# mct10/Speech-Vecalign

Measured on AMD Instinct MI355X. Metric: aligned doc-pairs/sec, higher is better.
Workload: dtype bf16; 1 GPU; synthetic 4096x4096 d=1024 bf16 embeddings, 4 overlap layers/side, 10 alignment types, band 14, coarse-to-fine (max_size_full_dp=300), 1024 doc-pairs per GPU per step; pipeline=1, N=4096, M=4096, d=1024, overlaps=4, parallelism=dp1 (pairs sharded, no collective)

## Files before the change

### include/svx.h

```cpp
#ifndef SVX_H
#define SVX_H

#include <stdint.h>

#ifdef __cplusplus
extern "C" {
#endif

typedef struct svx_ctx svx_ctx;

enum svx_dtype { SVX_F32 = 0, SVX_F16 = 1, SVX_BF16 = 2 };

enum svx_status {
    SVX_OK = 0,
    SVX_ERR_ARG = 1,
    SVX_ERR_OVERLAPS = 2,
    SVX_ERR_HIP = 3,
    SVX_ERR_TRACEBACK = 4,
    SVX_ERR_NOMEM = 5,
    SVX_ERR_EXTEND = 6,
    SVX_ERR_PATH = 7,
    SVX_ERR_BP = 8
};

#define SVX_MAX_LEVELS 16
#define SVX_MAX_TYPES 128
#define SVX_MAX_DIM 2048

int svx_create(int device_id, svx_ctx **out);
int svx_destroy(svx_ctx *ctx);
int svx_set_stream(svx_ctx *ctx, void *hip_stream);
int svx_synchronize(svx_ctx *ctx);
const char *svx_last_error(const svx_ctx *ctx);
const char *svx_version(void);
int64_t svx_scratch_bytes(const svx_ctx *ctx);


int svx_dense_costs(svx_ctx *ctx, const float *vecs0, int k0, int s0, const float *vecs1, int k1, int s1, int d,
                    const float *norm0, const float *norm1, int offset0, int offset1, float *costs);

int svx_dense_dp(svx_ctx *ctx, const float *cost, int s0, int s1, float pen, double *csum, int32_t *bp);

int svx_score_path(svx_ctx *ctx, const int32_t *xx, const int32_t *yy, int64_t n, const float *norm1,
                   const float *norm2, const float *vecs1, int rows1, const float *vecs2, int rows2, int d, float *out);

int svx_sparse_costs(svx_ctx *ctx, const float *vecs0, int k0, int xsize, const float *vecs1, int k1, int ysize,
                     int d, const float *norms0, const float *norms1, const int32_t *path, int A,
                     const int32_t *types_host, int T, int width_over2, float *costs, int32_t *b_offset);

int svx_sparse_dp(svx_ctx *ctx, const float *costs, const int32_t *b_offset_in, int A, int B,
                  const int32_t *types_host, int T, double del_penalty, int x_in_size, int y_in_size,
                  double *csum, int32_t *xp, int32_t *yp, int32_t *b_offset_out);


int svx_make_norm1(svx_ctx *ctx, float *vecs, int64_t rows, int d);

int svx_downsample(svx_ctx *ctx, const float *vecs, int k, int n, int d, float *half);

int svx_compute_norms(svx_ctx *ctx, const float *vecs0, int k0, int n0, const float *vecs1, int k1, int n1, int d,
                      const int32_t *idx, int samples_per_overlap, float *norms0);

int svx_del_penalty(svx_ctx *ctx, const float *scores, int64_t n, double frac, double *del_penalty);

int svx_dense_traceback(svx_ctx *ctx, const int32_t *bp, int s0, int s1, int32_t *align, int32_t *count);

int svx_sparse_traceback(svx_ctx *ctx, const double *csum, const int32_t *xp, const int32_t *yp,
                         const int32_t *b_offset_out, int a_out, int B, int xsize, int ysize, int32_t *align,
                         double *scores, int32_t *count);

int svx_search_path(svx_ctx *ctx, const int32_t *align, const int32_t *n_align, int upsample, int size0,
                    int size1, int32_t *path, int32_t *path_len);

int svx_gather_rows(svx_ctx *ctx, const void *table, int64_t n_rows, int d, int dtype, const int32_t *idx, int64_t n_out,
                    void *out);


int svx_mt19937_choice(uint32_t *key, int32_t *pos, int64_t n, int64_t size, int32_t *out);

int64_t svx_norm_index_count(int n, int m, int k0, int k1, int max_size_full_dp, int num_samps_for_norm, int have_norms0,
                             int have_norms1);
int64_t svx_knob_index_count(int n, int m, int max_size_full_dp, int costs_sample_size);

int svx_draw_indices(uint32_t *key, int32_t *pos, int n, int m, int k0, int k1, int max_size_full_dp, int costs_sample_size,
                     int num_samps_for_norm, int have_norms0, int have_norms1, int32_t *norm_idx, int32_t *knob_idx);

int svx_candidate_table(const char *seg_path, const char *cat_path, const char *ignore_path, int max_overlaps, int32_t *table,
                        int cap_lines, int32_t *n_lines, int64_t *n_candidates, char *err, int err_cap);

int64_t svx_format_alignments(const int32_t *rows, const double *scores, int64_t n, char *out, int64_t cap);


#define SVX_MARGIN_RATIO 0
#define SVX_MARGIN_DISTANCE 1
#define SVX_MARGIN_ABSOLUTE 2

int svx_unit_rows(svx_ctx *ctx, const void *rows, int dtype, int64_t n, int d, void *out, int out_dtype);

int svx_knn_mean_sim(svx_ctx *ctx, const void *queries, int q_dtype, int64_t n, const void *db, int db_dtype,
                     int64_t n_db, int d, int k, float *mean_sim);

int svx_knn_topk_merge(svx_ctx *ctx, const void *queries, int q_dtype, int64_t n, const void *db, int db_dtype,
                       int64_t n_db, int d, int k, float *topk, int first, float *mean_sim);

int svx_knn_search(svx_ctx *ctx, const void *queries, int q_dtype, int64_t n, const void *db, int db_dtype,
                   int64_t n_db, int d, int k, int64_t id_base, float *sims, int64_t *ids, int first);

int svx_margin_scores(svx_ctx *ctx, const void *x, const void *y, int dtype, int64_t n, int d, const float *mean_xy,
                      const float *mean_yx, int margin, float *scores);


int svx_knn_list_means(svx_ctx *ctx, const float *sims, int64_t n, int k, float *mean);

int svx_margin_candidates(svx_ctx *ctx, const float *sims, const int64_t *ids, int64_t n, int k, const float *mean_q,
                          const float *mean_db, int64_t n_db, int64_t id_base, int margin, float *scores, int64_t *best_id,
                          float *best_score);

int64_t svx_mine_greedy(const int64_t *order, int64_t n_cand, const int64_t *src, const int64_t *tgt, int64_t n_src,
                        int64_t n_tgt, int64_t *out);


typedef struct svx_align_params {
    int32_t dtype;
    int32_t d;
    int32_t n_types;
    int32_t types[2 * SVX_MAX_TYPES];
    int32_t width_over2;
    int32_t max_size_full_dp;
    int32_t costs_sample_size;
    int32_t num_samps_for_norm;
    double del_percentile_frac;
    int32_t search_mode;
    int32_t reserved0;
} svx_align_params;

#define SVX_SEARCH_COARSE_TO_FINE 0
// ... 54 lines not shown
```

### speech-vecalign_amd/csrc/svx_api.hip

```cpp
#include <stdarg.h>
#include <stdio.h>
#include <stdlib.h>
#include <string.h>

#include <chrono>
#include <functional>
#include <memory>
#include <type_traits>
#include <vector>

#include "svx_common.h"

static char g_err[512] = "";

int svx_fail(svx_ctx* ctx, int code, const char* fmt, ...) {
    char* dst = ctx ? ctx->err : g_err;
    va_list ap;
    va_start(ap, fmt);
    vsnprintf(dst, 512, fmt, ap);
    va_end(ap);
    return code;
}

static const char* kStageNames[] = {"pyr0",       "pyrN",     "pyr_aux",      "knob_scoresN", "knob",      "dense_costs",
// ... 277 lines not shown
        if (x < 1 || y < 1 || x > 100 || y > 100) return svx_fail(ctx, SVX_ERR_ARG, "alignment type (%d,%d): sizes must be >= 1", x, y);
        out->x[t] = (int8_t)x;
        out->y[t] = (int8_t)y;
        if (x + y > out->maxstep) out->maxstep = x + y;
    }
    out->x[T] = 0; out->y[T] = 1;
    out->x[T + 1] = 1; out->y[T + 1] = 0;
    return SVX_OK;
}

static int check_dim(svx_ctx* ctx, int d) {
    if (d <= 0 || d % 8 != 0 || d > SVX_MAX_DIM)
        return svx_fail(ctx, SVX_ERR_ARG, "embedding dimension %d: must be a positive multiple of 8, at most %d", d, SVX_MAX_DIM);
    return SVX_OK;
}

#define NEED(ctx, cond, ...) \
    do { if (!(cond)) return svx_fail(ctx, SVX_ERR_ARG, __VA_ARGS__); } while (0)

extern "C" {

int svx_dense_costs(svx_ctx* ctx, const float* vecs0, int k0, int s0, const float* vecs1, int k1, int s1, int d,
                    const float* norm0, const float* norm1, int offset0, int offset1, float* costs) {
    NEED(ctx, ctx && vecs0 && vecs1 && norm0 && norm1 && costs, "svx_dense_costs: null argument");
    NEED(ctx, k0 > offset0 && k1 > offset1 && offset0 >= 0 && offset1 >= 0, "svx_dense_costs: offsets (%d,%d) outside %d/%d layers", offset0, offset1, k0, k1);
    int rc = check_dim(ctx, d);
    if (rc) return rc;
    return svxl_dense_costs(ctx, vecs0 + (size_t)offset0 * s0 * d, s0, vecs1 + (size_t)offset1 * s1 * d, s1, d,
                            norm0 + (size_t)offset0 * s0, norm1 + (size_t)offset1 * s1, offset0 + 1, offset1 + 1, costs);
}

int svx_dense_dp(svx_ctx* ctx, const float* cost, int s0, int s1, float pen, double* csum, int32_t* bp) {
    NEED(ctx, ctx && bp && (cost || s0 == 0 || s1 == 0), "svx_dense_dp: null argument");
    NEED(ctx, s0 >= 0 && s1 >= 0, "svx_dense_dp: negative size");
    return svxl_dense_dp(ctx, cost, s0, s1, pen, csum, bp);
}

int svx_score_path(svx_ctx* ctx, const int32_t* xx, const int32_t* yy, int64_t n, const float* norm1, const float* norm2,
                   const float* vecs1, int rows1, const float* vecs2, int rows2, int d, float* out) {
    NEED(ctx, ctx && xx && yy && norm1 && norm2 && vecs1 && vecs2 && out, "svx_score_path: null argument");
    NEED(ctx, rows1 > 0 && rows2 > 0, "svx_score_path: empty vecs");
    int rc = check_dim(ctx, d);
    if (rc) return rc;
    return svxl_score_path(ctx, xx, yy, n, norm1, norm2, vecs1, rows1, vecs2, rows2, d, out);
}

int svx_sparse_costs(svx_ctx* ctx, const float* vecs0, int k0, int xsize, const float* vecs1, int k1, int ysize, int d,
                     const float* norms0, const float* norms1, const int32_t* path, int A, const int32_t* types_host, int T,
                     int width_over2, float* costs, int32_t* b_offset) {
    NEED(ctx, ctx && vecs0 && vecs1 && norms0 && norms1 && path && b_offset && (costs || T == 0), "svx_sparse_costs: null argument");
    NEED(ctx, width_over2 >= 1 && A >= 0, "svx_sparse_costs: bad width/path length");
    int rc = check_dim(ctx, d);
    if (rc) return rc;
    SvxTypes ty;
    rc = make_types(ctx, types_host, T, &ty);
    if (rc) return rc;
    int mx = 0, my = 0;
    for (int t = 0; t < T; t++) { if (ty.x[t] > mx) mx = ty.x[t]; if (ty.y[t] > my) my = ty.y[t]; }
    if (mx > k0) return svx_fail(ctx, SVX_ERR_OVERLAPS, "%d x overlaps requrested (via alignment_types), but vecs0 only has %d", mx, k0);
    if (my > k1) return svx_fail(ctx, SVX_ERR_OVERLAPS, "%d y overlaps requrested (via alignment_types), but vecs1 only has %d", my, k1);
    rc = arena_reserve(ctx, 256);
    if (rc) return rc;
    int* status = reinterpret_cast<int*>(ctx->arena);
    SVX_HIP(ctx, hipMemsetAsync(status, 0, sizeof(int), ctx->stream));
    rc = svxl_band_costs(ctx, vecs0, k0, xsize, vecs1, k1, ysize, d, SVX_F32, nullptr, nullptr, norms0, norms1, path, A, ty,
                         width_over2, costs, b_offset, status);
    if (rc) return rc;
    int hs = 0;
    SVX_HIP(ctx, hipMemcpyAsync(&hs, status, sizeof(int), hipMemcpyDeviceToHost, ctx->stream));
    SVX_HIP(ctx, hipStreamSynchronize(ctx->stream));
    if (hs != 0) return svx_fail(ctx, hs, "search path is not a unit-step lattice path starting at (0,0)");
    return SVX_OK;
}

int svx_sparse_dp(svx_ctx* ctx, const float* costs, const int32_t* b_offset_in, int A, int B, const int32_t* types_host,
                  int T, double del_penalty, int x_in_size, int y_in_size, double* csum, int32_t* xp, int32_t* yp,
                  int32_t* b_offset_out) {
    NEED(ctx, ctx && b_offset_in && csum && xp && yp && b_offset_out && (costs || T == 0), "svx_sparse_dp: null argument");
    NEED(ctx, A >= 1 && B >= 1, "svx_sparse_dp: empty cost band");
    SvxTypes ty;
    int rc = make_types(ctx, types_host, T, &ty);
    if (rc) return rc;
    return svxl_sparse_dp(ctx, costs, b_offset_in, A, B, ty, del_penalty, x_in_size, y_in_size, csum, xp, yp, b_offset_out);
}

int svx_make_norm1(svx_ctx* ctx, float* vecs, int64_t rows, int d) {
    NEED(ctx, ctx && (vecs || rows == 0), "svx_make_norm1: null argument");
    int rc = check_dim(ctx, d);
    if (rc) return rc;
    return svxl_make_norm1(ctx, vecs, rows, d);
}

int svx_downsample(svx_ctx* ctx, const float* vecs, int k, int n, int d, float* half) {
    NEED(ctx, ctx && vecs && (half || n < 2), "svx_downsample: null argument");
    int rc = check_dim(ctx, d);
    if (rc) return rc;
    const int h = n / 2;
    if (h <= 0 || k <= 0) return SVX_OK;
    const int nblk = (h + SVX_PYR_SLOTS - 1) / SVX_PYR_SLOTS;
    Bump b;
    size_t o_part = b.take((size_t)k * nblk * d * sizeof(float));
    size_t o_mean = b.take((size_t)k * d * sizeof(float));
    rc = arena_reserve(ctx, b.off);
    if (rc) return rc;
    float* part = reinterpret_cast<float*>(ctx->arena + o_part);
    float* mean = reinterpret_cast<float*>(ctx->arena + o_mean);
    if ((rc = svxl_pairsum(ctx, vecs, k, n, d, half, part, nblk))) return rc;
    if ((rc = svxl_colmean_plain(ctx, part, k, nblk, d, h, mean))) return rc;
    return svxl_sub_mean(ctx, half, k, h, d, mean);
}

int svx_compute_norms(svx_ctx* ctx, const float* vecs0, int k0, int n0, const float* vecs1, int k1, int n1, int d,
                      const int32_t* idx, int samples_per_overlap, float* norms0) {
    NEED(ctx, ctx && vecs0 && vecs1 && idx && norms0, "svx_compute_norms: null argument");
    NEED(ctx, n1 > 0 && samples_per_overlap > 0 && k1 > 0, "svx_compute_norms: nothing to sample");
    int rc = check_dim(ctx, d);
    if (rc) return rc;
    rc = arena_reserve(ctx, (size_t)d * sizeof(float) + 256);
    if (rc) return rc;
    float* rbar = reinterpret_cast<float*>(ctx->arena);
    if ((rc = svxl_sample_mean_plain(ctx, vecs1, k1, n1, d, idx, samples_per_overlap, rbar))) return rc;
    return svxl_norms_from_rbar(ctx, vecs0, (int64_t)k0 * n0, d, rbar, norms0);
}

int svx_del_penalty(svx_ctx* ctx, const float* scores, int64_t n, double frac, double* del_penalty) {
    NEED(ctx, ctx && scores && del_penalty && n > 0, "svx_del_penalty: null/empty argument");
    return svxl_del_penalty(ctx, scores, n, frac, del_penalty);
}

int svx_dense_traceback(svx_ctx* ctx, const int32_t* bp, int s0, int s1, int32_t* align, int32_t* count) {
    NEED(ctx, ctx && bp && align && count, "svx_dense_traceback: null argument");
    return svxl_dense_traceback(ctx, bp, s0, s1, align, count);
}

int svx_sparse_traceback(svx_ctx* ctx, const double* csum, const int32_t* xp, const int32_t* yp, const int32_t* b_offset_out,
                         int a_out, int B, int xsize, int ysize, int32_t* align, double* scores, int32_t* count) {
    NEED(ctx, ctx && csum && xp && yp && b_offset_out && align && scores && count, "svx_sparse_traceback: null argument");
    return svxl_sparse_traceback(ctx, csum, xp, yp, b_offset_out, a_out, B, xsize, ysize, align, scores, count);
}

int svx_search_path(svx_ctx* ctx, const int32_t* align, const int32_t* n_align, int upsample, int size0, int size1,
                    int32_t* path, int32_t* path_len) {
    NEED(ctx, ctx && align && n_align && path && path_len, "svx_search_path: null argument");
    return svxl_search_path(ctx, align, n_align, upsample, size0, size1, path, size0 + size1 + 4, path_len);
}

int svx_gather_rows(svx_ctx* ctx, const void* table, int64_t n_rows, int d, int dtype, const int32_t* idx, int64_t n_out, void* out) {
    NEED(ctx, ctx && table && idx && out, "svx_gather_rows: null argument");
    NEED(ctx, dtype == SVX_F32 || dtype == SVX_F16 || dtype == SVX_BF16, "svx_gather_rows: unknown dtype %d", dtype);
    int rc = check_dim(ctx, d);
    if (rc) return rc;
    return svxl_gather_rows(ctx, table, n_rows, d * (dtype == SVX_F32 ? 4 : 2), dtype, idx, n_out, out);
}

}

__global__ void k_init_batch(const SvxPairDev* pairs) {
    const SvxPairDev& P = pairs[blockIdx.x];
    if (threadIdx.x != 0) return;
    *P.status = 0;
    for (int l = 0; l <= P.L; l++) {
        if (P.lev[l].n_align) *P.lev[l].n_align = 0;
        if (P.lev[l].path_len) *P.lev[l].path_len = 0;
    }
    if (P.straight) {
        int* r = P.lev[0].align;
// ... 645 lines not shown
```

### speech-vecalign_amd/csrc/svx_common.h

```cpp
#pragma once
#include <hip/hip_runtime.h>
#include <stdint.h>
#include <stddef.h>
#include "../../include/svx.h"

#define SVX_WAVE 64

#ifndef SVX_PYR_SLOTS
#define SVX_PYR_SLOTS 32
#endif
#define SVX_BC_TA 32
#define SVX_BC_TAMAX 64
#define SVX_BC_TB 16
#define SVX_BC_ROWS 48

struct ElemF32 {
    using storage = float;
    static constexpr int VEC = 4;
    static constexpr int DT = SVX_F32;
};
struct ElemF16 {
    using storage = uint16_t;
    static constexpr int VEC = 8;
    static constexpr int DT = SVX_F16;
// ... 149 lines not shown
    int* kstart;
    double* pen;
    int* path;
    int* path_len;
    int* cstart;
    int* nchunks;
    float* costs;
    int* boff;
    double* csum;
    int* xp;
    int* yp;
    unsigned char* bpk;
    int* boff_out;
    int* align;
    int* n_align;
    double* scores;
};

struct SvxPairDev {
    const void* v[2];
    int K[2];
    int L;
    int d;
    int norm_override[2];
    float* dcost;
    float* ddot;
    int* dbp;
    int* status;
    int straight;
    int t_nd, t_cap;
    int* t_lo;
    int* t_cnt;
    int* t_pref;
    int* t_flag;
    SvxLevel lev[SVX_MAX_LEVELS];
};

struct SvxTypes {
    int n;
    int maxstep;
    int8_t x[SVX_MAX_TYPES + 2];
    int8_t y[SVX_MAX_TYPES + 2];
};

struct svx_ctx {
    int device;
    hipStream_t stream;
    char* arena;
    size_t arena_bytes;
    size_t arena_used;
    char err[512];
    int profiling;
};

int svx_fail(svx_ctx* ctx, int code, const char* fmt, ...);
#define SVX_HIP(ctx, call)                                                                     \
    do {                                                                                       \
        hipError_t e_ = (call);                                                                \
        if (e_ != hipSuccess) return svx_fail(ctx, SVX_ERR_HIP, "%s: %s", #call, hipGetErrorString(e_)); \
    } while (0)
#define SVX_LAUNCH_CHECK(ctx, name)                                                            \
    do {                                                                                       \
        hipError_t e_ = hipGetLastError();                                                     \
        if (e_ != hipSuccess) return svx_fail(ctx, SVX_ERR_HIP, "launch %s: %s", name, hipGetErrorString(e_)); \
    } while (0)

int svxl_make_norm1(svx_ctx*, float* vecs, int64_t rows, int d);
int svxl_pairsum(svx_ctx*, const float* vecs, int k, int n, int d, float* half, float* part, int nblk);
int svxl_colmean_plain(svx_ctx*, const float* part, int k, int nblk, int d, int count, float* mean);
int svxl_sub_mean(svx_ctx*, float* half, int k, int h, int d, const float* mean);
int svxl_sample_mean_plain(svx_ctx*, const float* vecs, int k, int n, int d, const int* idx, int S, float* rbar);
int svxl_norms_from_rbar(svx_ctx*, const float* vecs, int64_t rows, int d, const float* rbar, float* norms);
int svxl_gather_rows(svx_ctx*, const void* table, long long n_rows, int row_bytes, int dtype, const int* idx, long long n_out, void* out);
int svxl_pyramid_level(svx_ctx*, const SvxPairDev* pairs, int n_pairs, int level, int dtype, int d, int max_nblk,
                       int max_ksum, int part);
int svxl_score_path(svx_ctx*, const int* xx, const int* yy, int64_t n, const float* n1, const float* n2,
                    const float* v1, int rows1, const float* v2, int rows2, int d, float* out);
int svxl_knob_scores(svx_ctx*, const SvxPairDev* pairs, int n_pairs, int max_levels, int max_kn, int max_n0, int dtype, int d,
                     int part);
int svxl_dense_costs(svx_ctx*, const float* v0, int s0, const float* v1, int s1, int d, const float* n0,
                     const float* n1, int mul0, int mul1, float* costs);
int svxl_dense_costs_batch(svx_ctx*, const SvxPairDev* pairs, int n_pairs, int max_s0, int max_s1, int dtype, int d);
int svxl_knob_from_dots(svx_ctx*, const SvxPairDev* pairs, int n_pairs, int max_kn);
int svxl_band_costs(svx_ctx*, const void* v0, int k0, int n, const void* v1, int k1, int m, int d, int dtype,
                    const float* inv0, const float* inv1, const float* nrm0, const float* nrm1, const int* path,
                    int A, const SvxTypes& types, int W, float* costs, int* boff, int* status);
int svxl_band_costs_batch(svx_ctx*, const SvxPairDev* pairs, int n_pairs, int depth, int max_A, const SvxTypes& types,
                          int W, int dtype, int d);
bool svxl_band2_limits(const SvxTypes& types, int W, int depth, int dtype, int d, int* lim, int* tamax);
int svxl_band_costs2_batch(svx_ctx*, const SvxPairDev* pairs, int n_pairs, int depth, int max_A, const SvxTypes& types, int W,
                           int dtype, int d);
int svxl_band_tiles_shape(const SvxTypes& types);
size_t svxl_band_tiles_scratch(const SvxTypes& types);
int svxl_band_tiles_batch(svx_ctx*, const SvxPairDev* pairs, int n_pairs, const SvxTypes& types, int W, int dtype, int max_nd,
                          int* gpref, int* ticket, float* planes);
int svxl_dense_dp(svx_ctx*, const float* cost, int s0, int s1, float pen, double* csum, int* bp);
int svxl_dense_stage_batch(svx_ctx*, const SvxPairDev* pairs, int n_pairs, int max_s0);
int svxl_dense_traceback(svx_ctx*, const int* bp, int s0, int s1, int* align, int* count);
int svxl_sparse_dp(svx_ctx*, const float* costs, const int* boff_in, int A, int B, const SvxTypes& types, double pen,
                   int xs, int ys, double* csum, int* xp, int* yp, int* boff_out);
int svxl_sparse_dp_batch(svx_ctx*, const SvxPairDev* pairs, int n_pairs, int depth, const SvxTypes& types, int B);
int svxl_sparse_traceback(svx_ctx*, const double* csum, const int* xp, const int* yp, const int* boff, int a_out,
                          int B, int xs, int ys, int* align, double* scores, int* count);
int svxl_sparse_traceback_batch(svx_ctx*, const SvxPairDev* pairs, int n_pairs, int depth, int B, int max_A, int packed);
int svxl_search_path(svx_ctx*, const int* align, const int* n_align, int upsample, int size0, int size1, int* path,
                     int cap, int* path_len);
int svxl_search_path_batch(svx_ctx*, const SvxPairDev* pairs, int n_pairs, int depth, int max_rows, int max_src_rows, int chunk_lim,
                           int chunk_tamax);
int svxl_del_penalty(svx_ctx*, const float* scores, int64_t n, double frac, double* out);
int svxl_del_penalty_batch(svx_ctx*, const SvxPairDev* pairs, int n_pairs, int max_levels, double frac);
```

### speech-vecalign_amd/csrc/svx_costs.hip

```cpp
#include <stdlib.h>

#include "svx_common.h"

namespace {

typedef __attribute__((ext_vector_type(8))) __bf16 bf16x8_t;
typedef __attribute__((ext_vector_type(8))) _Float16 f16x8_t;
typedef __attribute__((ext_vector_type(4))) float f32x4_t;

constexpr int RS = 144;

template <typename E>
struct Mma;
template <>
struct Mma<ElemBF16> {
    static constexpr int KS = 64, NK = 2, KSTEP_BYTES = 64;
    using frag = uint4;
    __device__ static __forceinline__ int lane_off(int lane) { return (lane & 15) * RS + 16 * (lane >> 4); }
    __device__ static __forceinline__ frag load(const char* p) { return *reinterpret_cast<const uint4*>(p); }
    __device__ static __forceinline__ void mma(f32x4_t& acc, const frag& a, const frag& b) {
        acc = __builtin_amdgcn_mfma_f32_16x16x32_bf16(__builtin_bit_cast(bf16x8_t, a), __builtin_bit_cast(bf16x8_t, b), acc, 0, 0, 0);
    }
};
template <>
// ... 115 lines not shown
    dense_block<E>(g, blockIdx.x, blockIdx.y, smem);
}

template <typename E, bool LV0>
__global__ __launch_bounds__(256) void k_dense_costs_batch(const SvxPairDev* __restrict__ pairs) {
    extern __shared__ __attribute__((aligned(16))) char smem[];
    const SvxPairDev& P = pairs[blockIdx.z];
    if ((P.L == 0) != LV0) return;
    const SvxLevel& Lv = P.lev[P.L];
    DenseArgs g;
    g.s0 = Lv.n[0];
    g.s1 = Lv.n[1];
    if ((int)blockIdx.x * DT >= g.s0 || (int)blockIdx.y * DT >= g.s1) return;
    g.d = P.d;
    g.v0 = LV0 ? P.v[0] : (const void*)Lv.P[0];
    g.v1 = LV0 ? P.v[1] : (const void*)Lv.P[1];
    g.inv0 = LV0 ? Lv.inv[0] : nullptr;
    g.inv1 = LV0 ? Lv.inv[1] : nullptr;
    g.n0 = Lv.nrm[0];
    g.n1 = Lv.nrm[1];
    g.mul0 = 1;
    g.mul1 = 1;
    g.costs = P.dcost;
    g.dots = LV0 ? nullptr : P.ddot;
    dense_block<E>(g, blockIdx.x, blockIdx.y, smem);
}

template <typename E, int NCH>
__device__ __forceinline__ float row_dot(const typename E::storage* a, const typename E::storage* b, int d, int lane) {
    float s = 0.f;
#pragma unroll
    for (int c = 0; c < NCH; c++) {
        const int col = (c * SVX_WAVE + lane) * E::VEC;
        if (col < d) {
            float x[E::VEC], y[E::VEC];
            load_piece<E>(a + col, x);
            load_piece<E>(b + col, y);
#pragma unroll
            for (int i = 0; i < E::VEC; i++) s += x[i] * y[i];
        }
    }
    return wave_sum(s);
}

struct ScoreArgs {
    const void* v1;
    const void* v2;
    const float* inv1;
    const float* inv2;
    const float* n1;
    const float* n2;
    const int* xx;
    const int* yy;
    int64_t n;
    int rows1, rows2, d;
    float* out;
};

template <typename E, int NCH>
__device__ void score_block(const ScoreArgs& g, int64_t first, int64_t stride) {
    using S = typename E::storage;
    const int lane = threadIdx.x & 63;
    for (int64_t i = first; i < g.n; i += stride) {
        int xi = g.xx[i], yi = g.yy[i];
        xi = xi < 0 ? 0 : (xi >= g.rows1 ? g.rows1 - 1 : xi);
        yi = yi < 0 ? 0 : (yi >= g.rows2 ? g.rows2 - 1 : yi);
        float dot = row_dot<E, NCH>(reinterpret_cast<const S*>(g.v1) + (size_t)xi * g.d,
                                    reinterpret_cast<const S*>(g.v2) + (size_t)yi * g.d, g.d, lane);
        if (lane == 0) {
            if (g.inv1) dot = dot * g.inv1[xi] * g.inv2[yi];
            const float den = g.n1[xi] + g.n2[yi];
            g.out[i] = (float)((2.0 * (1.0 - (double)dot)) / (double)den);
        }
    }
}

template <typename E, int NCH>
__global__ __launch_bounds__(256) void k_score_path(ScoreArgs g) {
    score_block<E, NCH>(g, (int64_t)blockIdx.x * 4 + (threadIdx.x >> 6), (int64_t)gridDim.x * 4);
}

__device__ __forceinline__ unsigned xcd_remap(unsigned id, unsigned n);

__global__ __launch_bounds__(256) void k_knob_sort(const SvxPairDev* __restrict__ pairs) {
    extern __shared__ __attribute__((aligned(16))) char smem[];
    __shared__ int part[256];
    const SvxPairDev& P = pairs[blockIdx.y];
    const int level = blockIdx.x;
    if (level > P.L) return;
    if (P.L >= 1 && level == P.L) return;
    const SvxLevel& Lv = P.lev[level];
    const int n = Lv.n[0], kn = Lv.kn, tid = threadIdx.x;
    int* cnt = reinterpret_cast<int*>(smem);
    for (int i = tid; i < n; i += 256) cnt[i] = 0;
    __syncthreads();
    for (int i = tid; i < kn; i += 256) {
        int x = Lv.kx[i];
        x = x < 0 ? 0 : (x >= n ? n - 1 : x);
        atomicAdd(&cnt[x], 1);
    }
    __syncthreads();
    const int per = (n + 255) / 256;
    const int lo = tid * per, hi = (lo + per) < n ? (lo + per) : n;
    int sum = 0;
    for (int i = lo; i < hi; i++) sum += cnt[i];
    part[tid] = sum;
    __syncthreads();
    if (tid == 0) {
        int run = 0;
        for (int i = 0; i < 256; i++) { const int v = part[i]; part[i] = run; run += v; }
    }
    __syncthreads();
    int run = part[tid];
    for (int i = lo; i < hi; i++) {
        const int v = cnt[i];
        cnt[i] = run;
        Lv.kstart[i] = run;
        run += v;
    }
    if (tid == 0) Lv.kstart[n] = kn;
    __syncthreads();
    for (int i = tid; i < kn; i += 256) {
        int x = Lv.kx[i];
        x = x < 0 ? 0 : (x >= n ? n - 1 : x);
        const int pos = atomicAdd(&cnt[x], 1);
        const int m = Lv.n[1];
        int y = Lv.ky[i];
        y = y < 0 ? 0 : (y >= m ? m - 1 : y);
        Lv.korder[pos] = i;
        Lv.kys[pos] = y;
    }
}

constexpr int KNOB_PF = 2;

template <typename E, int NCH, bool LV0>
__global__ __launch_bounds__(256) void k_knob_scores(const SvxPairDev* __restrict__ pairs, int nlev, int bpt) {
    using S = typename E::storage;
    constexpr int EPL = NCH * E::VEC;
    const unsigned wg = xcd_remap(blockIdx.x, gridDim.x);
    const int task = wg / bpt, blk = wg % bpt;
    const SvxPairDev& P = pairs[task / nlev];
    const int level = task % nlev + (LV0 ? 0 : 1);
    if (level > P.L) return;
    if (!LV0 && level == P.L) return;
    const SvxLevel& Lv = P.lev[level];
    const int lane = threadIdx.x & 63;
    const int n = Lv.n[0], d = P.d;
    const S* v1 = LV0 ? reinterpret_cast<const S*>(P.v[0]) : reinterpret_cast<const S*>(Lv.P[0]);
    const S* v2 = LV0 ? reinterpret_cast<const S*>(P.v[1]) : reinterpret_cast<const S*>(Lv.P[1]);
    const float* inv1 = LV0 ? Lv.inv[0] : nullptr;
    const float* inv2 = LV0 ? Lv.inv[1] : nullptr;
    for (int x = blk * 4 + (threadIdx.x >> 6); x < n; x += bpt * 4) {
        const int s0 = gld(Lv.kstart + x), s1 = gld(Lv.kstart + x + 1);
        if (s0 >= s1) continue;
        float xr[EPL];
#pragma unroll
        for (int c = 0; c < NCH; c++) {
            const int col = (c * SVX_WAVE + lane) * E::VEC;
            if (col < d) {
                gload_piece<E>(v1 + (size_t)x * d + col, xr + c * E::VEC);
            } else {
#pragma unroll
                for (int i = 0; i < E::VEC; i++) xr[c * E::VEC + i] = 0.f;
            }
        }
        const float nx = gld(Lv.nrm[0] + x);
        const float ix = LV0 ? gld(inv1 + x) : 1.0f;
        constexpr int PF = KNOB_PF;
        const int ns = s1 - s0;
        for (int cb = 0; cb < ns; cb += SVX_WAVE) {
            const int cn = min(SVX_WAVE, ns - cb);
            const int ys_l = lane < cn ? gld(Lv.kys + s0 + cb + lane) : 0;
            const int is_l = lane < cn ? gld(Lv.korder + s0 + cb + lane) : 0;
            const float nrm_l = lane < cn ? gld(Lv.nrm[1] + ys_l) : 0.f;
            const float inv_l = (LV0 && lane < cn) ? gld(inv2 + ys_l) : 1.f;
            float dots_l = 0.f;
            uint4 yraw[PF][NCH];
#pragma unroll
            for (int u = 0; u < PF; u++) {
                const int yu = __builtin_amdgcn_readlane(ys_l, u);
#pragma unroll
                for (int c = 0; c < NCH; c++) {
                    const int col = (c * SVX_WAVE + lane) * E::VEC;
                    yraw[u][c] = (u < cn && col < d) ? gld16(v2 + (size_t)yu * d + col) : make_uint4(0, 0, 0, 0);
                }
            }
            for (int base = 0; base < cn; base += PF) {
#pragma unroll
                for (int u = 0; u < PF; u++) {
                    const int k = base + u;
                    if (k >= cn) break;
                    float dot = 0.f;
#pragma unroll
                    for (int c = 0; c < NCH; c++) {
                        float yr[E::VEC];
                        decode_piece<E>(yraw[u][c], yr);
#pragma unroll
                        for (int e = 0; e < E::VEC; e++) dot += xr[c * E::VEC + e] * yr[e];
                    }
                    if (k + PF < cn) {
                        const int yn = __builtin_amdgcn_readlane(ys_l, k + PF);
#pragma unroll
                        for (int c = 0; c < NCH; c++) {
                            const int col = (c * SVX_WAVE + lane) * E::VEC;
                            yraw[u][c] = col < d ? gld16(v2 + (size_t)yn * d + col) : make_uint4(0, 0, 0, 0);
                        }
                    }
                    dot = wave_sum(dot);
                    dots_l = lane == k ? dot : dots_l;
                }
            }
            if (lane < cn) {
                float dot = dots_l;
// ... 370 lines not shown
    const int a0 = Lv.cstart[chunk_a], TAe = Lv.cstart[chunk_a + 1] - a0;
    g.n = Lv.n[0];
    g.m = Lv.n[1];
    g.d = P.d;
    g.v0 = LV0 ? P.v[0] : (const void*)Lv.P[0];
    g.v1 = LV0 ? P.v[1] : (const void*)Lv.P[1];
    g.inv0 = LV0 ? Lv.inv[0] : nullptr;
    g.inv1 = LV0 ? Lv.inv[1] : nullptr;
    g.nrm0 = Lv.nrm[0];
    g.nrm1 = Lv.nrm[1];
    g.path = Lv.path;
    g.W = W;
    g.costs = Lv.costs;
    g.boff = Lv.boff;
    g.status = P.status;
    g.atb = 1;
    band_block<E, NPT, SW>(g, ty, kx, ky, a0, TAe, item % nchunk_b, smem);
}

inline int nch_f32(int d) {
    int c = (d + 255) / 256;
    return c <= 1 ? 1 : c <= 2 ? 2 : c <= 4 ? 4 : 8;
}
inline int nch_16(int d) {
    int c = (d + 511) / 512;
    return c <= 1 ? 1 : c <= 2 ? 2 : 4;
}

constexpr size_t DENSE_SMEM = 2 * DT * sizeof(char*) + 2 * DT * RS;

}

int svxl_dense_costs(svx_ctx* ctx, const float* v0, int s0, const float* v1, int s1, int d, const float* n0,
                     const float* n1, int mul0, int mul1, float* costs) {
    if (s0 <= 0 || s1 <= 0) return SVX_OK;
    DenseArgs g{v0, v1, s0, s1, d, nullptr, nullptr, n0, n1, mul0, mul1, costs, nullptr};
    hipLaunchKernelGGL(k_dense_costs<ElemF32>, dim3((s0 + DT - 1) / DT, (s1 + DT - 1) / DT), dim3(256), DENSE_SMEM, ctx->stream, g);
    SVX_LAUNCH_CHECK(ctx, "k_dense_costs");
    return SVX_OK;
}

int svxl_dense_costs_batch(svx_ctx* ctx, const SvxPairDev* pairs, int n_pairs, int max_s0, int max_s1, int dtype, int d) {
    (void)d;
    if (n_pairs <= 0 || max_s0 <= 0 || max_s1 <= 0) return SVX_OK;
    dim3 grid((max_s0 + DT - 1) / DT, (max_s1 + DT - 1) / DT, n_pairs);
    hipLaunchKernelGGL((k_dense_costs_batch<ElemF32, false>), grid, dim3(256), DENSE_SMEM, ctx->stream, pairs);
    if (dtype == SVX_F32)
        hipLaunchKernelGGL((k_dense_costs_batch<ElemF32, true>), grid, dim3(256), DENSE_SMEM, ctx->stream, pairs);
    else if (dtype == SVX_F16)
        hipLaunchKernelGGL((k_dense_costs_batch<ElemF16, true>), grid, dim3(256), DENSE_SMEM, ctx->stream, pairs);
    else
        hipLaunchKernelGGL((k_dense_costs_batch<ElemBF16, true>), grid, dim3(256), DENSE_SMEM, ctx->stream, pairs);
    SVX_LAUNCH_CHECK(ctx, "k_dense_costs_batch");
    return SVX_OK;
}

int svxl_score_path(svx_ctx* ctx, const int* xx, const int* yy, int64_t n, const float* n1, const float* n2,
                    const float* v1, int rows1, const float* v2, int rows2, int d, float* out) {
    if (n <= 0) return SVX_OK;
    ScoreArgs g{v1, v2, nullptr, nullptr, n1, n2, xx, yy, n, rows1, rows2, d, out};
    int64_t nb = (n + 3) / 4;
    if (nb > 16384) nb = 16384;
#define M(N) hipLaunchKernelGGL((k_score_path<ElemF32, N>), dim3((unsigned)nb), dim3(256), 0, ctx->stream, g)
    switch (nch_f32(d)) {
        case 1: M(1); break;
        case 2: M(2); break;
        case 4: M(4); break;
        default: M(8); break;
    }
#undef M
    SVX_LAUNCH_CHECK(ctx, "k_score_path");
    return SVX_OK;
}

int svxl_knob_from_dots(svx_ctx* ctx, const SvxPairDev* pairs, int n_pairs, int max_kn) {
    if (n_pairs <= 0 || max_kn <= 0) return SVX_OK;
    int nb = (max_kn + 255) / 256;
    if (nb > 16) nb = 16;
    hipLaunchKernelGGL(k_knob_from_dots, dim3(nb, n_pairs), dim3(256), 0, ctx->stream, pairs);
    SVX_LAUNCH_CHECK(ctx, "k_knob_from_dots");
    return SVX_OK;
}

int svxl_knob_scores(svx_ctx* ctx, const SvxPairDev* pairs, int n_pairs, int max_L, int max_kn, int max_n0, int dtype, int d,
                     int part) {
    if (n_pairs <= 0 || max_kn <= 0) return SVX_OK;
    hipStream_t st = ctx->stream;
    const bool unsorted = (size_t)(max_n0 + 1) * sizeof(int) > 150 * 1024;
    if (unsorted) {
        if (part == 0) return SVX_OK;
        const int nbu = (max_kn + 3) / 4 < 2048 ? (max_kn + 3) / 4 : 2048;
#define U32(N, LV0, GY) hipLaunchKernelGGL((k_knob_scores_unsorted<ElemF32, N, LV0>), dim3(nbu, GY, n_pairs), dim3(256), 0, st, pairs)
#define U16(E, N) hipLaunchKernelGGL((k_knob_scores_unsorted<E, N, true>), dim3(nbu, 1, n_pairs), dim3(256), 0, st, pairs)
        if (part == 1) {
            if (max_L >= 1) {
                switch (nch_f32(d)) {
                    case 1: U32(1, false, max_L); break;
                    case 2: U32(2, false, max_L); break;
                    case 4: U32(4, false, max_L); break;
                    default: U32(8, false, max_L); break;
                }
            }
        } else if (dtype == SVX_F32) {
            switch (nch_f32(d)) {
                case 1: U32(1, true, 1); break;
                case 2: U32(2, true, 1); break;
                case 4: U32(4, true, 1); break;
                default: U32(8, true, 1); break;
            }
        } else if (dtype == SVX_F16) {
            switch (nch_16(d)) {
                case 1: U16(ElemF16, 1); break;
                case 2: U16(ElemF16, 2); break;
                default: U16(ElemF16, 4); break;
            }
        } else {
            switch (nch_16(d)) {
                case 1: U16(ElemBF16, 1); break;
                case 2: U16(ElemBF16, 2); break;
                default: U16(ElemBF16, 4); break;
            }
        }
#undef U32
#undef U16
        SVX_LAUNCH_CHECK(ctx, "k_knob_scores_unsorted");
        return SVX_OK;
    }
    if (part == 0) {
        const size_t smem = (size_t)(max_n0 + 1) * sizeof(int);
        if (smem > 64 * 1024)
            SVX_HIP(ctx, hipFuncSetAttribute((const void*)k_knob_sort, hipFuncAttributeMaxDynamicSharedMemorySize, (int)smem));
        hipLaunchKernelGGL(k_knob_sort, dim3(max_L + 1, n_pairs), dim3(256), smem, st, pairs);
        SVX_LAUNCH_CHECK(ctx, "k_knob_sort");
        return SVX_OK;
    }
    int nb = (max_n0 + 3) / 4;
    if (nb > 1024) nb = 1024;
#define M32(N, LV0, GY) hipLaunchKernelGGL((k_knob_scores<ElemF32, N, LV0>), dim3((unsigned)nb * (GY) * n_pairs), dim3(256), 0, st, pairs, GY, nb)
#define M16(E, N) hipLaunchKernelGGL((k_knob_scores<E, N, true>), dim3((unsigned)nb * n_pairs), dim3(256), 0, st, pairs, 1, nb)
    if (part == 1 && max_L >= 1) {
        switch (nch_f32(d)) {
            case 1: M32(1, false, max_L); break;
            case 2: M32(2, false, max_L); break;
            case 4: M32(4, false, max_L); break;
            default: M32(8, false, max_L); break;
        }
    }
    if (part != 2) {
    } else if (dtype == SVX_F32) {
        switch (nch_f32(d)) {
            case 1: M32(1, true, 1); break;
            case 2: M32(2, true, 1); break;
            case 4: M32(4, true, 1); break;
            default: M32(8, true, 1); break;
        }
    } else if (dtype == SVX_F16) {
        switch (nch_16(d)) {
            case 1: M16(ElemF16, 1); break;
            case 2: M16(ElemF16, 2); break;
            default: M16(ElemF16, 4); break;
        }
    } else {
        switch (nch_16(d)) {
            case 1: M16(ElemBF16, 1); break;
            case 2: M16(ElemBF16, 2); break;
            default: M16(ElemBF16, 4); break;
        }
    }
#undef M32
#undef M16
    SVX_LAUNCH_CHECK(ctx, "k_knob_scores");
    return SVX_OK;
}

static int types_layers(const SvxTypes& ty, int* kx, int* ky) {
    int mx = 0, my = 0;
    for (int t = 0; t < ty.n; t++) {
        if (ty.x[t] > mx) mx = ty.x[t];
        if (ty.y[t] > my) my = ty.y[t];
    }
    *kx = mx;
    *ky = my;
    return 0;
}

struct BandPlan {
    int sw, npt;
    size_t smem;
};

static int band_plan(svx_ctx* ctx, int kx, int ky, int ntypes, BandPlan* bp) {
    const int NR = (kx + ky) * ROWS;
    const char* sw_env = getenv("SVX_BAND_SW");
    const int sw_max = sw_env ? atoi(sw_env) : 4;
    for (int sw = 4; sw >= 1; sw >>= 1) {
        if (sw > sw_max) continue;
        const int tpp = sw == 4 ? BC_WAVES / 3 : TPP_FULL;
        const int ntp = ntypes < tpp ? ntypes : tpp;
        if (sw == 4 && ntypes > tpp) continue;
        const BandLds L = band_lds(kx, ky, sw, ntp);
        const int npt = (NR * 8 * sw + BC_THREADS - 1) / BC_THREADS;
        if (sw == 4 && (NR > 2 * ROWS || L.total > 64 * 1024)) continue;
        if (sw == 2 && (L.total > 128 * 1024 || npt > 12)) continue;
        if (L.total > 160 * 1024 || npt > 14)
            return svx_fail(ctx, SVX_ERR_ARG, "band costs: %d+%d overlap layers need %zu bytes of LDS / %d staging pieces (limits 160 KiB / 14)",
                            kx, ky, L.total, npt);
        bp->sw = sw;
        bp->npt = npt < 1 ? 1 : npt;
        bp->smem = L.total;
        return SVX_OK;
    }
    return svx_fail(ctx, SVX_ERR_ARG, "band costs: no launch configuration");
// ... 92 lines not shown
```

### speech-vecalign_amd/svx/_lib.py

```python
import ctypes
import os
import threading

_HERE = os.path.dirname(os.path.abspath(__file__))
LIB_PATH = os.environ.get("SVX_LIB") or os.path.join(_HERE, "libsvx.so")

SVX_F32, SVX_F16, SVX_BF16 = 0, 1, 2
SVX_MAX_TYPES = 128
SVX_MAX_LEVELS = 16
SVX_MARGIN_RATIO, SVX_MARGIN_DISTANCE, SVX_MARGIN_ABSOLUTE = 0, 1, 2
SVX_SEARCH_COARSE_TO_FINE, SVX_SEARCH_STRAIGHT = 0, 1

SVX_OK, SVX_ERR_ARG, SVX_ERR_OVERLAPS, SVX_ERR_HIP, SVX_ERR_TRACEBACK = 0, 1, 2, 3, 4
SVX_ERR_NOMEM, SVX_ERR_EXTEND, SVX_ERR_PATH, SVX_ERR_BP = 5, 6, 7, 8

DEVICE_ERRORS = {
    SVX_ERR_TRACEBACK: "traceback bug",
    SVX_ERR_BP: "got unknown value",
    SVX_ERR_EXTEND: "asked to extend alignments but already bigger than requested",
    SVX_ERR_PATH: "search path is not a unit-step lattice path",
}

c_int, c_i64, c_f32, c_f64, c_vp = ctypes.c_int, ctypes.c_int64, ctypes.c_float, ctypes.c_double, ctypes.c_void_p


class AlignParams(ctypes.Structure):
    _fields_ = [
        ("dtype", ctypes.c_int32),
        ("d", ctypes.c_int32),
        ("n_types", ctypes.c_int32),
        ("types", ctypes.c_int32 * (2 * SVX_MAX_TYPES)),
        ("width_over2", ctypes.c_int32),
        ("max_size_full_dp", ctypes.c_int32),
        ("costs_sample_size", ctypes.c_int32),
        ("num_samps_for_norm", ctypes.c_int32),
        ("del_percentile_frac", ctypes.c_double),
        ("search_mode", ctypes.c_int32),
        ("reserved0", ctypes.c_int32),
    ]


class LevelView(ctypes.Structure):
    _fields_ = [
        ("size0", ctypes.c_int32), ("size1", ctypes.c_int32), ("k0", ctypes.c_int32), ("k1", ctypes.c_int32),
        ("n_types", ctypes.c_int32), ("band", ctypes.c_int32), ("path_len", ctypes.c_int32), ("n_align", ctypes.c_int32),
        ("n0", c_vp), ("n1", c_vp), ("del_penalty", c_vp), ("searchpath", c_vp), ("a_b_costs", c_vp), ("b_offset", c_vp),
        ("a_b_csum", c_vp), ("a_b_bp", c_vp), ("a_b_xp", c_vp), ("a_b_yp", c_vp), ("new_b_offset", c_vp),
        ("alignments", c_vp), ("alignment_scores", c_vp),
        ("costs_1to1", c_vp), ("x_y_tb_diag", c_vp), ("v0_l0", c_vp), ("v1_l0", c_vp),
        ("knob_scores", c_vp), ("n_knob", ctypes.c_int32), ("reserved", ctypes.c_int32),
    ]


class Pair(ctypes.Structure):
    _fields_ = [
        ("vecs0", c_vp), ("vecs1", c_vp),
        ("n", ctypes.c_int32), ("m", ctypes.c_int32), ("k0", ctypes.c_int32), ("k1", ctypes.c_int32),
        ("norm_idx", c_vp), ("knob_idx", c_vp),
        ("norms0", c_vp), ("norms1", c_vp),
        ("align", c_vp), ("scores", c_vp), ("info", c_vp), ("del_pen", c_vp),
    ]


_SIGS = {
    "svx_create": (c_int, [c_int, ctypes.POINTER(c_vp)]),
    "svx_destroy": (c_int, [c_vp]),
    "svx_set_stream": (c_int, [c_vp, c_vp]),
    "svx_synchronize": (c_int, [c_vp]),
    "svx_last_error": (ctypes.c_char_p, [c_vp]),
    "svx_version": (ctypes.c_char_p, []),
    "svx_scratch_bytes": (c_i64, [c_vp]),
    "svx_dense_costs": (c_int, [c_vp, c_vp, c_int, c_int, c_vp, c_int, c_int, c_int, c_vp, c_vp, c_int, c_int, c_vp]),
    "svx_dense_dp": (c_int, [c_vp, c_vp, c_int, c_int, c_f32, c_vp, c_vp]),
    "svx_score_path": (c_int, [c_vp, c_vp, c_vp, c_i64, c_vp, c_vp, c_vp, c_int, c_vp, c_int, c_int, c_vp]),
    "svx_sparse_costs": (c_int, [c_vp, c_vp, c_int, c_int, c_vp, c_int, c_int, c_int, c_vp, c_vp, c_vp, c_int,
                                 ctypes.POINTER(ctypes.c_int32), c_int, c_int, c_vp, c_vp]),
    "svx_sparse_dp": (c_int, [c_vp, c_vp, c_vp, c_int, c_int, ctypes.POINTER(ctypes.c_int32), c_int, c_f64, c_int, c_int,
                              c_vp, c_vp, c_vp, c_vp]),
    "svx_make_norm1": (c_int, [c_vp, c_vp, c_i64, c_int]),
    "svx_downsample": (c_int, [c_vp, c_vp, c_int, c_int, c_int, c_vp]),
    "svx_compute_norms": (c_int, [c_vp, c_vp, c_int, c_int, c_vp, c_int, c_int, c_int, c_vp, c_int, c_vp]),
    "svx_del_penalty": (c_int, [c_vp, c_vp, c_i64, c_f64, c_vp]),
    "svx_dense_traceback": (c_int, [c_vp, c_vp, c_int, c_int, c_vp, c_vp]),
    "svx_sparse_traceback": (c_int, [c_vp, c_vp, c_vp, c_vp, c_vp, c_int, c_int, c_int, c_int, c_vp, c_vp, c_vp]),
    "svx_search_path": (c_int, [c_vp, c_vp, c_vp, c_int, c_int, c_int, c_vp, c_vp]),
    "svx_gather_rows": (c_int, [c_vp, c_vp, c_i64, c_int, c_int, c_vp, c_i64, c_vp]),
    "svx_unit_rows": (c_int, [c_vp, c_vp, c_int, c_i64, c_int, c_vp, c_int]),
    "svx_knn_mean_sim": (c_int, [c_vp, c_vp, c_int, c_i64, c_vp, c_int, c_i64, c_int, c_int, c_vp]),
    "svx_knn_topk_merge": (c_int, [c_vp, c_vp, c_int, c_i64, c_vp, c_int, c_i64, c_int, c_int, c_vp, c_int, c_vp]),
    "svx_knn_search": (c_int, [c_vp, c_vp, c_int, c_i64, c_vp, c_int, c_i64, c_int, c_int, c_i64, c_vp, c_vp, c_int]),
    "svx_margin_scores": (c_int, [c_vp, c_vp, c_vp, c_int, c_i64, c_int, c_vp, c_vp, c_int, c_vp]),
    "svx_knn_list_means": (c_int, [c_vp, c_vp, c_i64, c_int, c_vp]),
    "svx_margin_candidates": (c_int, [c_vp, c_vp, c_vp, c_i64, c_int, c_vp, c_vp, c_i64, c_i64, c_int, c_vp, c_vp, c_vp]),
    "svx_mine_greedy": (c_i64, [c_vp, c_i64, c_vp, c_vp, c_i64, c_i64, c_vp]),
    "svx_mt19937_choice": (c_int, [c_vp, ctypes.POINTER(ctypes.c_int32), c_i64, c_i64, c_vp]),
    "svx_norm_index_count": (c_i64, [c_int, c_int, c_int, c_int, c_int, c_int, c_int, c_int]),
    "svx_knob_index_count": (c_i64, [c_int, c_int, c_int, c_int]),
    "svx_draw_indices": (c_int, [c_vp, ctypes.POINTER(ctypes.c_int32), c_int, c_int, c_int, c_int, c_int, c_int, c_int, c_int, c_int,
                                 c_vp, c_vp]),
    "svx_candidate_table": (c_int, [ctypes.c_char_p, ctypes.c_char_p, ctypes.c_char_p, c_int, c_vp, c_int,
                                    ctypes.POINTER(ctypes.c_int32), ctypes.POINTER(c_i64), ctypes.c_char_p, c_int]),
    "svx_format_alignments": (c_i64, [c_vp, c_vp, c_i64, c_vp, c_i64]),
    "svx_num_levels": (c_int, [c_int, c_int, c_int]),
    "svx_knob_count": (c_i64, [c_int, c_int, c_int]),
    "svx_align_batch": (c_int, [c_vp, ctypes.POINTER(AlignParams), ctypes.POINTER(Pair), c_int]),
    "svx_debug_level": (c_int, [c_vp, c_int, c_int, ctypes.POINTER(LevelView)]),
    "svx_copy_to_host": (c_int, [c_vp, c_vp, c_vp, c_i64]),
    "svx_set_profiling": (c_int, [c_vp, c_int]),
    "svx_set_pipeline": (c_int, [c_vp, c_int]),
    "svx_flush": (c_int, [c_vp]),
    "svx_stage_ms": (c_f64, [c_vp, ctypes.c_char_p]),
    "svx_stage_launches": (c_int, [c_vp, ctypes.c_char_p]),
}

EXPORTS = tuple(_SIGS)

_lib = None
_lock = threading.Lock()


def load():
    global _lib
    with _lock:
        if _lib is None:
            if not os.path.exists(LIB_PATH):
                raise ImportError(
                    "libsvx.so not found at %s: build it with `make -C speech-vecalign_amd/csrc` "
                    "(there is no CPU fallback)" % LIB_PATH)
            L = ctypes.CDLL(LIB_PATH)
            for name, (res, args) in _SIGS.items():
                fn = getattr(L, name)
                fn.restype = res
                fn.argtypes = args
            _lib = L
    return _lib


class SvxError(Exception):
    def __init__(self, code, msg):
        super().__init__(msg)
        self.code = code


class Context:

    def __init__(self, device=0):
        import torch
        if not torch.cuda.is_available():
            raise RuntimeError("svx needs a HIP device (torch.cuda.is_available() is False); there is no CPU fallback")
        self.lib = load()
        self.device = int(device)
        h = c_vp()
        rc = self.lib.svx_create(self.device, ctypes.byref(h))
        if rc != 0:
            raise SvxError(rc, self.lib.svx_last_error(None).decode())
        self.h = h
        self.torch = torch
        self.tdev = torch.device("cuda", self.device)
        self.pipeline = False
        self._held = []
        if os.environ.get("SVX_PIPELINE") == "1":
# ... 57 lines not shown
```

Before: 9666 doc-pairs/s.

## Rewrite knob counting sort with register-resident ranks and wave-parallel prefix scan

After: 9721 doc-pairs/s, median of 6. About the same (+0.6%).

```diff
diff --git a/include/svx.h b/include/svx.h
--- a/include/svx.h
+++ b/include/svx.h
@@ -51,6 +51,9 @@
 int svx_sparse_dp(svx_ctx *ctx, const float *costs, const int32_t *b_offset_in, int A, int B,
                   const int32_t *types_host, int T, double del_penalty, int x_in_size, int y_in_size,
                   double *csum, int32_t *xp, int32_t *yp, int32_t *b_offset_out);
+
+int svx_knob_sort(svx_ctx *ctx, const int32_t *kx, const int32_t *ky, int kn, int n, int m, int32_t *korder,
+                  int32_t *kys, int32_t *kstart);
 
 
 int svx_make_norm1(svx_ctx *ctx, float *vecs, int64_t rows, int d);
diff --git a/speech-vecalign_amd/csrc/svx_api.hip b/speech-vecalign_amd/csrc/svx_api.hip
--- a/speech-vecalign_amd/csrc/svx_api.hip
+++ b/speech-vecalign_amd/csrc/svx_api.hip
@@ -383,6 +383,13 @@
     int rc = make_types(ctx, types_host, T, &ty);
     if (rc) return rc;
     return svxl_sparse_dp(ctx, costs, b_offset_in, A, B, ty, del_penalty, x_in_size, y_in_size, csum, xp, yp, b_offset_out);
+}
+
+int svx_knob_sort(svx_ctx* ctx, const int32_t* kx, const int32_t* ky, int kn, int n, int m, int32_t* korder, int32_t* kys,
+                  int32_t* kstart) {
+    NEED(ctx, ctx && kstart && ((kx && ky && korder && kys) || kn == 0), "svx_knob_sort: null argument");
+    NEED(ctx, kn >= 0 && n >= 1 && m >= 1, "svx_knob_sort: %d samples over %d x %d rows", kn, n, m);
+    return svxl_knob_sort(ctx, kx, ky, kn, n, m, korder, kys, kstart);
 }
 
 int svx_make_norm1(svx_ctx* ctx, float* vecs, int64_t rows, int d) {
diff --git a/speech-vecalign_amd/csrc/svx_common.h b/speech-vecalign_amd/csrc/svx_common.h
--- a/speech-vecalign_amd/csrc/svx_common.h
+++ b/speech-vecalign_amd/csrc/svx_common.h
@@ -255,6 +255,7 @@
                      const float* n1, int mul0, int mul1, float* costs);
 int svxl_dense_costs_batch(svx_ctx*, const SvxPairDev* pairs, int n_pairs, int max_s0, int max_s1, int dtype, int d);
 int svxl_knob_from_dots(svx_ctx*, const SvxPairDev* pairs, int n_pairs, int max_kn);
+int svxl_knob_sort(svx_ctx*, const int* kx, const int* ky, int kn, int n, int m, int* korder, int* kys, int* kstart);
 int svxl_band_costs(svx_ctx*, const void* v0, int k0, int n, const void* v1, int k1, int m, int d, int dtype,
                     const float* inv0, const float* inv1, const float* nrm0, const float* nrm1, const int* path,
                     int A, const SvxTypes& types, int W, float* costs, int* boff, int* status);
diff --git a/speech-vecalign_amd/csrc/svx_costs.hip b/speech-vecalign_amd/csrc/svx_costs.hip
--- a/speech-vecalign_amd/csrc/svx_costs.hip
+++ b/speech-vecalign_amd/csrc/svx_costs.hip
@@ -221,54 +221,139 @@
 
 __device__ __forceinline__ unsigned xcd_remap(unsigned id, unsigned n);
 
-__global__ __launch_bounds__(256) void k_knob_sort(const SvxPairDev* __restrict__ pairs) {
+constexpr int KS_RES = 80;
+constexpr int KS_YB = 20;
+constexpr int KS_BATCH = 16;
+constexpr size_t KNOB_SORT_MAX_LDS = 150 * 1024;
+static_assert(KNOB_SORT_MAX_LDS / sizeof(int) <= 65536 && 256 * KS_RES <= 32768 && KS_RES % KS_YB == 0, "x and rank share a register");
+
+__host__ __device__ constexpr size_t knob_sort_lds(int n) { return (size_t)((n + 4) & ~3) * sizeof(int); }
+
+__device__ __forceinline__ int clamp_row(int v, int n) { return v < 0 ? 0 : (v >= n ? n - 1 : v); }
+
+__device__ __forceinline__ void knob_sort_block(const int* __restrict__ kx, const int* __restrict__ ky, int kn, int n, int m,
+                                                int* __restrict__ korder, int* __restrict__ kys, int* __restrict__ kstart,
+                                                int* cnt) {
+    __shared__ int wtot[2][4];
+    const int tid = threadIdx.x, lane = tid & 63, wave = tid >> 6;
+    const int nres = kn < 256 * KS_RES ? kn : 256 * KS_RES;
+    const int jfull = nres >> 8;
+    const bool tail = tid + 256 * jfull < nres;
+#define KS_HAS(j) ((j) < jfull || ((j) == jfull && tail))
+    int xr[KS_RES];
+#pragma unroll
+    for (int j = 0; j < KS_RES; j++)
+        xr[j] = KS_HAS(j) ? gld(kx + (tid + 256 * j)) : 0;
+    const int n4 = (n + 4) & ~3;
+    for (int i = tid; i < n4; i += 256) cnt[i] = 0;
+    __syncthreads();
+#pragma unroll
+    for (int j = 0; j < KS_RES; j++) {
+        const int x = clamp_row(xr[j], n);
+        xr[j] = KS_HAS(j) ? x | (atomicAdd(&cnt[x], 1) << 16) : 0;
+    }
+    if (kn > nres) {
+        __syncthreads();
+        for (int b = nres; b < kn; b += 256 * KS_BATCH) {
+            int xb[KS_BATCH];
+#pragma unroll
+            for (int j = 0; j < KS_BATCH; j++) {
+                const int i = b + tid + 256 * j;
+                xb[j] = i < kn ? gld(kx + i) : 0;
+            }
+#pragma unroll
+            for (int j = 0; j < KS_BATCH; j++)
+                if (b + tid + 256 * j < kn) atomicAdd(&cnt[clamp_row(xb[j], n)], 1);
+        }
+    }
+    __syncthreads();
+    int carry = 0;
+    for (int base = 0, it = 0; base < n4; base += 1024, it ^= 1) {
+        const int e = base + tid * 4;
+        int4 v = make_int4(0, 0, 0, 0);
+        if (e < n4) v = *reinterpret_cast<const int4*>(cnt + e);
+        const int s = v.x + v.y + v.z + v.w;
+        int inc = s;
+#pragma unroll
+        for (int o = 1; o < SVX_WAVE; o <<= 1) {
+            const int t = __shfl_up(inc, o);
+            if (lane >= o) inc += t;
+        }
+        if (lane == SVX_WAVE - 1) wtot[it][wave] = inc;
+        __syncthreads();
+        int before = 0, total = 0;
+#pragma unroll
+        for (int w = 0; w < 4; w++) {
+            const int t = wtot[it][w];
+            before += w < wave ? t : 0;
+            total += t;
+        }
+        if (e < n4) {
+            int4 o;
+            o.x = carry + before + inc - s;
+            o.y = o.x + v.x;
+            o.z = o.y + v.y;
+            o.w = o.z + v.z;
+            *reinterpret_cast<int4*>(cnt + e) = o;
+        }
+        carry += total;
+    }
+    __syncthreads();
+    for (int i = tid; i <= n; i += 256) gst(kstart + i, cnt[i]);
+#pragma unroll
+    for (int c = 0; c < KS_RES; c += KS_YB) {
+        int yb[KS_YB];
+#pragma unroll
+        for (int j = 0; j < KS_YB; j++) yb[j] = KS_HAS(c + j) ? gld(ky + (tid + 256 * (c + j))) : 0;
+#pragma unroll
+        for (int j = 0; j < KS_YB; j++) {
+            const int i = tid + 256 * (c + j);
+            if (KS_HAS(c + j)) {
+                const int pos = cnt[xr[c + j] & 0xffff] + (xr[c + j] >> 16);
+                gst(korder + pos, i);
+                gst(kys + pos, clamp_row(yb[j], m));
+            }
+        }
+    }
+    if (kn > nres) {
+        __syncthreads();
+        for (int b = nres; b < kn; b += 256 * KS_BATCH) {
+            int xb[KS_BATCH], yb[KS_BATCH];
+#pragma unroll
+            for (int j = 0; j < KS_BATCH; j++) {
+                const int i = b + tid + 256 * j;
+                xb[j] = i < kn ? gld(kx + i) : 0;
+                yb[j] = i < kn ? gld(ky + i) : 0;
+            }
+#pragma unroll
+            for (int j = 0; j < KS_BATCH; j++) {
+                const int i = b + tid + 256 * j;
+                if (i < kn) {
+                    const int pos = atomicSub(&cnt[clamp_row(xb[j], n) + 1], 1) - 1;
+                    gst(korder + pos, i);
+                    gst(kys + pos, clamp_row(yb[j], m));
+                }
+            }
+        }
+    }
+}
+
+#undef KS_HAS
+
+__global__ __launch_bounds__(256) __attribute__((amdgpu_waves_per_eu(3))) void k_knob_sort(const SvxPairDev* __restrict__ pairs) {
     extern __shared__ __attribute__((aligned(16))) char smem[];
-    __shared__ int part[256];
     const SvxPairDev& P = pairs[blockIdx.y];
     const int level = blockIdx.x;
     if (level > P.L) return;
     if (P.L >= 1 && level == P.L) return;
     const SvxLevel& Lv = P.lev[level];
-    const int n = Lv.n[0], kn = Lv.kn, tid = threadIdx.x;
-    int* cnt = reinterpret_cast<int*>(smem);
-    for (int i = tid; i < n; i += 256) cnt[i] = 0;
-    __syncthreads();
-    for (int i = tid; i < kn; i += 256) {
-        int x = Lv.kx[i];
-        x = x < 0 ? 0 : (x >= n ? n - 1 : x);
-        atomicAdd(&cnt[x], 1);
-    }
-    __syncthreads();
-    const int per = (n + 255) / 256;
-    const int lo = tid * per, hi = (lo + per) < n ? (lo + per) : n;
-    int sum = 0;
-    for (int i = lo; i < hi; i++) sum += cnt[i];
-    part[tid] = sum;
-    __syncthreads();
-    if (tid == 0) {
-        int run = 0;
-        for (int i = 0; i < 256; i++) { const int v = part[i]; part[i] = run; run += v; }
-    }
-    __syncthreads();
-    int run = part[tid];
-    for (int i = lo; i < hi; i++) {
-        const int v = cnt[i];
-        cnt[i] = run;
-        Lv.kstart[i] = run;
-        run += v;
-    }
-    if (tid == 0) Lv.kstart[n] = kn;
-    __syncthreads();
-    for (int i = tid; i < kn; i += 256) {
-        int x = Lv.kx[i];
-        x = x < 0 ? 0 : (x >= n ? n - 1 : x);
-        const int pos = atomicAdd(&cnt[x], 1);
-        const int m = Lv.n[1];
-        int y = Lv.ky[i];
-        y = y < 0 ? 0 : (y >= m ? m - 1 : y);
-        Lv.korder[pos] = i;
-        Lv.kys[pos] = y;
-    }
+    knob_sort_block(Lv.kx, Lv.ky, Lv.kn, Lv.n[0], Lv.n[1], Lv.korder, Lv.kys, Lv.kstart, reinterpret_cast<int*>(smem));
+}
+
+__global__ __launch_bounds__(256) __attribute__((amdgpu_waves_per_eu(3))) void k_knob_sort_one(const int* __restrict__ kx, const int* __restrict__ ky, int kn, int n, int m,
+                                                       int* __restrict__ korder, int* __restrict__ kys, int* __restrict__ kstart) {
+    extern __shared__ __attribute__((aligned(16))) char smem[];
+    knob_sort_block(kx, ky, kn, n, m, korder, kys, kstart, reinterpret_cast<int*>(smem));
 }
 
 constexpr int KNOB_PF = 2;
@@ -805,11 +890,22 @@
     return SVX_OK;
 }
 
+int svxl_knob_sort(svx_ctx* ctx, const int* kx, const int* ky, int kn, int n, int m, int* korder, int* kys, int* kstart) {
+    if ((size_t)(n + 1) * sizeof(int) > KNOB_SORT_MAX_LDS)
+        return svx_fail(ctx, SVX_ERR_ARG, "svx_knob_sort: the histogram of %d rows does not fit LDS", n);
+    const size_t smem = knob_sort_lds(n);
+    if (smem > 64 * 1024)
+        SVX_HIP(ctx, hipFuncSetAttribute((const void*)k_knob_sort_one, hipFuncAttributeMaxDynamicSharedMemorySize, (int)smem));
+    hipLaunchKernelGGL(k_knob_sort_one, dim3(1), dim3(256), smem, ctx->stream, kx, ky, kn, n, m, korder, kys, kstart);
+    SVX_LAUNCH_CHECK(ctx, "k_knob_sort_one");
+    return SVX_OK;
+}
+
 int svxl_knob_scores(svx_ctx* ctx, const SvxPairDev* pairs, int n_pairs, int max_L, int max_kn, int max_n0, int dtype, int d,
                      int part) {
     if (n_pairs <= 0 || max_kn <= 0) return SVX_OK;
     hipStream_t st = ctx->stream;
-    const bool unsorted = (size_t)(max_n0 + 1) * sizeof(int) > 150 * 1024;
+    const bool unsorted = (size_t)(max_n0 + 1) * sizeof(int) > KNOB_SORT_MAX_LDS;
     if (unsorted) {
         if (part == 0) return SVX_OK;
         const int nbu = (max_kn + 3) / 4 < 2048 ? (max_kn + 3) / 4 : 2048;
@@ -850,7 +946,7 @@
         return SVX_OK;
     }
     if (part == 0) {
-        const size_t smem = (size_t)(max_n0 + 1) * sizeof(int);
+        const size_t smem = knob_sort_lds(max_n0);
         if (smem > 64 * 1024)
             SVX_HIP(ctx, hipFuncSetAttribute((const void*)k_knob_sort, hipFuncAttributeMaxDynamicSharedMemorySize, (int)smem));
         hipLaunchKernelGGL(k_knob_sort, dim3(max_L + 1, n_pairs), dim3(256), smem, st, pairs);
diff --git a/speech-vecalign_amd/svx/_lib.py b/speech-vecalign_amd/svx/_lib.py
--- a/speech-vecalign_amd/svx/_lib.py
+++ b/speech-vecalign_amd/svx/_lib.py
@@ -77,6 +77,7 @@
                                  ctypes.POINTER(ctypes.c_int32), c_int, c_int, c_vp, c_vp]),
     "svx_sparse_dp": (c_int, [c_vp, c_vp, c_vp, c_int, c_int, ctypes.POINTER(ctypes.c_int32), c_int, c_f64, c_int, c_int,
                               c_vp, c_vp, c_vp, c_vp]),
+    "svx_knob_sort": (c_int, [c_vp, c_vp, c_vp, c_int, c_int, c_int, c_vp, c_vp, c_vp]),
     "svx_make_norm1": (c_int, [c_vp, c_vp, c_i64, c_int]),
     "svx_downsample": (c_int, [c_vp, c_vp, c_int, c_int, c_int, c_vp]),
     "svx_compute_norms": (c_int, [c_vp, c_vp, c_int, c_int, c_vp, c_int, c_int, c_int, c_vp, c_int, c_vp]),
```
